# 0beqz/realism-effects

Measured on AMD Instinct MI355X. Metric: Mpixels/s SSGI+denoise @4K steps=20; achieved HBM GB/s vs peak, higher is better.
Workload: dtype f32; 1 GPU; configs[2]: 3840x2160 (8.29 Mpixel) on one GPU, steps=20 refineSteps=5 denoiseIterations=1, K1+K2+2xK3+K4 per step; frame=3840x2160, tile_rows=2160, halo_rows=0, direct_light=True, half_store=rtz, uv_model=reference_gl, parallelism=single GPU

## Files before the change

### realism-effects_amd/csrc/k1_ssgi.hip

```cpp
#include "rfx_brdf.h"
#include "rfx_kernels.h"

namespace {

constexpr int BASE = 16;
constexpr int K1_TH = 1;
typedef uint32_t k1_cell_t;
constexpr int K1_WAVES = 8;
constexpr int K1_COUNTERS = 64;
constexpr int K1_TABLE_CELLS = 9216;
RFX_DEV uint32_t k1_half_toward(float v, bool up) {
    uint32_t h = rfx_f2h_rne(v) & 0xffffu;
    const float f = rfx_h2f((unsigned short)h);
    if (up ? (f < v) : (f > v)) {
        const bool neg = (h & 0x8000u) != 0;
        if (up) h = neg ? (h == 0x8000u ? 0x0001u : h - 1u) : h + 1u;
        else h = neg ? h + 1u : (h == 0x0000u ? 0x8001u : h - 1u);
    }
    return h;
}
RFX_DEV k1_cell_t k1_cell_pack(float mn, float mx) { return k1_half_toward(mn, false) | (k1_half_toward(mx, true) << 16); }
RFX_DEV float2 k1_cell_load(const k1_cell_t *t, unsigned int i) {
    const uint32_t v = *(const k1_cell_t *)((const char *)t + i);
    return make_float2(rfx_h2f((unsigned short)(v & 0xffffu)), rfx_h2f((unsigned short)(v >> 16)));
// ... 599 lines not shown

__global__ __launch_bounds__(256) void k1_hit_mask(FrameDims d, int y0, int y1, TexView depth, TexViewW out, const float4 *hits, int allow_missed, unsigned int *mask) {
    const int x = blockIdx.x * 64 + threadIdx.x, y = y0 + blockIdx.y * 4 + threadIdx.y;
    d.viol = 0;
    if (x >= d.W || y >= y1) return;
    const float dp = ((const float *)depth.ptr)[rfx_xy_index(d, depth.row0, depth.rows, x, y)];
    if (dp == 1.0f) return;
    const size_t i = (size_t)rfx_local_row(d, out.row0, out.rows, y) * d.W + x;
    const float4 h0 = hits[2 * i], h1 = hits[2 * i + 1];
    const float u[2] = {h0.x, h0.z}, v[2] = {h0.y, h0.w}, px[2] = {h1.x, h1.y};
#pragma unroll
    for (int r = 0; r < 2; r++) {
        const bool missed = px[r] == 10.0e9f;
        if ((allow_missed || !missed) && u[r] >= 0.0f && u[r] <= 1.0f && v[r] >= 0.0f && v[r] <= 1.0f) {
            const int row = rfx_nearest_idx(v[r], d.fH, d.H), col = rfx_nearest_idx(u[r], d.fW, d.W);
            const unsigned int bit = 1u << ((unsigned int)(col * 32) / (unsigned int)d.W);
            if (!(mask[row] & bit)) atomicOr(&mask[row], bit);
        }
    }
}

template <int VEC>
__global__ __launch_bounds__(256) void k1_prepare(const float *depth, float *viewz, float2 *base, int W, int H, int base_w, float nearMulFar,
                                                   float farMinusNear, float cameraFar, float nearMinusFar, float cameraNear, int perspective) {
    static_assert(VEC == 1 || VEC == 4, "one texel or one aligned float4 per lane and row");
    const int x0 = (blockIdx.x * 64 + threadIdx.x) * VEC, cy = blockIdx.y * 4 + threadIdx.y, y0 = cy * BASE;
    if (y0 >= H) return;
    float mn = INFINITY, mx = -INFINITY;
    float d[BASE][VEC];
    const bool in_x = x0 < W;
#pragma unroll
    for (int r = 0; r < BASE; r++) {
        const int y = y0 + r;
#pragma unroll
        for (int k = 0; k < VEC; k++) d[r][k] = 1.0f;
        if (in_x && y < H) {
            if (VEC == 4) {
                const float4 t = *(const float4 *)(depth + (size_t)y * W + x0);
                d[r][0] = t.x; d[r][1] = t.y; d[r][2] = t.z; d[r][3] = t.w;
            } else {
                d[r][0] = depth[(size_t)y * W + x0];
            }
        }
    }
#pragma unroll
    for (int r = 0; r < BASE; r++) {
        const int y = y0 + r;
        if (in_x && y < H) {
            float z[VEC];
#pragma unroll
            for (int k = 0; k < VEC; k++) {
                z[k] = perspective ? nearMulFar / (farMinusNear * d[r][k] - cameraFar) : d[r][k] * nearMinusFar - cameraNear;
                mn = fminf(mn, z[k]);
                mx = fmaxf(mx, z[k]);
            }
            if (VEC == 4) *(float4 *)(viewz + (size_t)y * W + x0) = make_float4(z[0], z[1], z[2], z[3]);
            else viewz[(size_t)y * W + x0] = z[0];
        }
    }
#pragma unroll
    for (int o = 1; o < BASE / VEC; o <<= 1) {
        mn = fminf(mn, __shfl_xor(mn, o));
        mx = fmaxf(mx, __shfl_xor(mx, o));
    }
    const int cx = x0 / BASE;
    if ((threadIdx.x & (BASE / VEC - 1)) == 0 && cx < base_w) base[(size_t)cy * base_w + cx] = make_float2(mn, mx);
}

__global__ __launch_bounds__(256) void k1_pack_cells(const float2 *base, int base_w, int base_h, k1_cell_t *cells, int cells_w, int cells_h, int cells_pitch, int up,
                                                     int cells_padded, unsigned int *tile_counter) {
    const int i = blockIdx.x * 256 + threadIdx.x;
    if (i < 64) tile_counter[i * 32] = 0u;
    if (i >= cells_padded) return;
    const int cy = i / cells_pitch, cx = i - cy * cells_pitch;
    if (cy >= cells_h || cx >= cells_w) {
        cells[i] = 0u;
        return;
    }
    float mn = INFINITY, mx = -INFINITY;
    for (int by = cy << up; by < min((cy + 1) << up, base_h); by++)
        for (int bx = cx << up; bx < min((cx + 1) << up, base_w); bx++) {
            const float2 b = base[(size_t)by * base_w + bx];
            mn = fminf(mn, b.x);
            mx = fmaxf(mx, b.y);
        }
    cells[i] = k1_cell_pack(mn, mx);
}

__global__ __launch_bounds__(256) void k1_env_mip(const float4 *src, float4 *dst, int sw, int sh, int dw, int dh, int to_half, int rtz) {
// ... 22 lines not shown
    hipLaunchKernelGGL(k1_env_mip, grid, block, 0, stream, src, dst, sw, sh, dw, dh, to_half ? 1 : 0, rtz ? 1 : 0);
    return hipGetLastError();
}

int rfx_k1_base_cell() { return BASE; }

hipError_t rfx_launch_k1_hit_rows(const FrameDims &d, int y0, int y1, TexView depth, TexViewW out, const float4 *hits, bool allow_missed, int *rows, hipStream_t stream) {
    dim3 block(64, 4), grid((d.W + 63) / 64, (y1 - y0 + 3) / 4);
    hipLaunchKernelGGL(k1_hit_rows, grid, block, 0, stream, d, y0, y1, depth, out, hits, allow_missed ? 1 : 0, rows);
    return hipGetLastError();
}

hipError_t rfx_launch_k1_hit_mask(const FrameDims &d, int y0, int y1, TexView depth, TexViewW out, const float4 *hits, bool allow_missed, unsigned int *mask, hipStream_t stream) {
    dim3 block(64, 4), grid((d.W + 63) / 64, (y1 - y0 + 3) / 4);
    hipLaunchKernelGGL(k1_hit_mask, grid, block, 0, stream, d, y0, y1, depth, out, hits, allow_missed ? 1 : 0, mask);
    return hipGetLastError();
}

hipError_t rfx_launch_k1_prepare(const K1Args &A, hipStream_t stream) {
    const int W = A.dims.W, H = A.dims.H;
    const dim3 block(64, 4);
    if (W % 4 == 0 && ((uintptr_t)A.depth.ptr & 15u) == 0 && ((uintptr_t)A.viewz & 15u) == 0)
        hipLaunchKernelGGL(k1_prepare<4>, dim3((W + 255) / 256, ((H + BASE - 1) / BASE + 3) / 4), block, 0, stream, (const float *)A.depth.ptr, A.viewz, A.coarse, W, H, A.coarse_w,
                           A.nearMulFar, A.farMinusNear, A.p.camera.far_, A.nearMinusFar, A.p.camera.near_, A.p.camera.isPerspective);
    else
        hipLaunchKernelGGL(k1_prepare<1>, dim3((W + 63) / 64, ((H + BASE - 1) / BASE + 3) / 4), block, 0, stream, (const float *)A.depth.ptr, A.viewz, A.coarse, W, H, A.coarse_w,
                           A.nearMulFar, A.farMinusNear, A.p.camera.far_, A.nearMinusFar, A.p.camera.near_, A.p.camera.isPerspective);
    int up = 0;
    while ((BASE << up) < (1 << A.cell_shift)) up++;
    const int padded = A.cells_vec4 * 4;
    hipLaunchKernelGGL(k1_pack_cells, dim3((padded + 255) / 256), dim3(256), 0, stream, (const float2 *)A.coarse, A.coarse_w, A.coarse_h,
                       (k1_cell_t *)A.cells, A.cells_w, A.cells_h, A.cells_pitch, up, padded, A.tile_counter);
    return hipGetLastError();
}

hipError_t rfx_launch_k1(const K1Args &A, int stage, hipStream_t stream) {
    const int nbx = (A.out_w + 63) / 64, nby = (A.y1 - A.y0 + K1_TH - 1) / K1_TH;
    const int want = (nbx * nby + K1_WAVES - 1) / K1_WAVES, n_cu = A.n_cu > 0 ? A.n_cu : 256;
    dim3 block(64 * K1_WAVES), grid(1);
    const float *P = A.p.camera.projectionMatrix;
    const bool persp = P[1] == 0.f && P[2] == 0.f && P[3] == 0.f && P[4] == 0.f && P[6] == 0.f && P[7] == 0.f && P[12] == 0.f && P[13] == 0.f &&
                       P[15] == 0.f && P[11] == -1.f;
    const bool env = A.p.useEnvMap != 0, mis = env && A.p.importanceSampling != 0;
#define K1_GO_S(P, E, M, S)                                                                                                   \
    do {                                                                                                                      \
        static int per_cu[64] = {0};                                                                                          \
        int dev = 0;                                                                                                          \
        hipGetDevice(&dev);                                                                                                   \
        int nb = (dev >= 0 && dev < 64) ? per_cu[dev] : 0;                                                                    \
        if (nb <= 0) {                                                                                                        \
// ... 27 lines not shown
```

### realism-effects_amd/csrc/k3_denoise.hip

```cpp
#include <type_traits>
#include "rfx_device.h"
#include "rfx_kernels.h"
#include "k3_rotation_table.h"

namespace {

constexpr int TW = 64, TH = 8;
constexpr int NT = TW * TH;
static_assert(TW % 64 == 0 && NT <= 1024, "a tile row is whole wavefronts; at most 16 wavefronts per workgroup");
constexpr int K3_XCD_G = 1;
constexpr int K3_LDS_MAX = 80 * 1024;

struct CenterTexel {
    float3 rgb;
    float a;
    float lumaPow;
    float w;
    float total;
};

RFX_DEV float k3_logc(float x) { return rfx_log2(x); }
RFX_DEV float k3_unlog(float o) { return rfx_exp2(o) - 1.0f; }
RFX_DEV float k3_luma(float3 a) {
    return rfx_exp2(__builtin_fmaf(0.125f, rfx_log2(rfx_lum(a)), 0.125f * -0.5287663729448977f));
// ... 22 lines not shown
    const rfx_f2 d = c.lumaPow - tapLuma;
    const rfx_f2 lumaDiff = k3_f2(fminf(fabsf(d.x), 0.5f), fminf(fabsf(d.y), 0.5f));
    const rfx_f2 e = l2w - lumaDiff * lumaPhiL2;
    const rfx_f2 wl = k3_f2(rfx_exp2(e.x), rfx_exp2(e.y));
    rfx_f2 w = (wl * c.omw + disocclW * c.w) * c.w;
    w = k3_f2((w.x < 0.0001f) ? 0.0f : w.x, (w.y < 0.0001f) ? 0.0f : w.y);
    c.r += tr * w;
    c.g += tg * w;
    c.b += tb * w;
    c.total += w;
}
RFX_DEV rfx_f2 k3_logc2(rfx_f2 x) {
    const rfx_f2 x1 = x + 1.0f;
    return k3_f2(rfx_log2(x1.x), rfx_log2(x1.y));
}
RFX_DEV rfx_f2 k3_luma2(rfx_f2 r, rfx_f2 g, rfx_f2 b) {
    const rfx_f2 lum = 0.2125f * r + 0.7154f * g + 0.0721f * b;
    const rfx_f2 l = k3_f2(rfx_log2(lum.x), rfx_log2(lum.y));
    const rfx_f2 e = 0.125f * l + (0.125f * -0.5287663729448977f);
    return k3_f2(rfx_exp2(e.x), rfx_exp2(e.y));
}


template <bool IN_TEMPORAL, int TC, int PITCH, bool WHOLE>
RFX_DEV void k3_tiled_body(const K3Args &A, const FrameDims &d) {
    constexpr bool PAIR = TC == 2;
    extern __shared__ float4 lds[];
    const int Rx = A.tile.Rx, Ry = A.tile.Ry, LW = A.tile.LW, LH = A.tile.LH;
    const int ntex = PITCH * LH;
    float4 *s_geom = lds;
    float4 *s_in0 = lds + ntex;
    uint2 *s_inN = reinterpret_cast<uint2 *>(lds + ntex);
    uint4 *s_in2 = reinterpret_cast<uint4 *>(lds + ntex);
    float *s_depth = reinterpret_cast<float *>(lds + ntex) + (IN_TEMPORAL ? 8 : 4) * (size_t)ntex;
    const int skip = (PAIR && IN_TEMPORAL) ? A.tile.skip : 0;
    if (PAIR && IN_TEMPORAL && skip > 0) {
        const int nal = ntex - 2 * skip;
        s_depth = reinterpret_cast<float *>(lds) + 4 - skip;
        s_geom = lds + 1 + nal / 4 - skip;
        s_in0 = lds + 1 + nal / 4 + nal - 2 * skip;
    }
    const rfx_denoise_params &p = A.p;
    if (PAIR && IN_TEMPORAL && skip > 0) {
        const int t = threadIdx.y * TW + threadIdx.x, nal = ntex - 2 * skip;
        float *f = reinterpret_cast<float *>(lds);
        if (t < 4) f[t] = 0.0f;
        if (t < 8 * skip) f[4 + nal * 13 + t] = 0.0f;
    }
    const TileXY tile = rfx_xcd_tile<K3_XCD_G>((d.W + TW - 1) / TW, (A.y1 - A.y0 + TH - 1) / TH);
    if (!tile.valid) return;
    const int tx0 = tile.bx * TW, ty0 = A.y0 + tile.by * TH;
    const int tid = threadIdx.y * TW + threadIdx.x;
    const float *depthp = (const float *)A.depth.ptr;
    const uint4 *gbp = (const uint4 *)A.gbuffer.ptr;

    const float invLW = 1.0f / (float)LW;
    for (int i = tid; i < LW * LH; i += NT) {
        const int ly = (int)(((float)i + 0.5f) * invLW), lx = i - __mul24(ly, LW);
        const int li = __mul24(ly, PITCH) + lx;
        if (li < skip || li >= ntex - skip) continue;
        const int uy = ty0 - Ry + ly;
        if (uy > A.y1 - 1 + Ry) continue;
        const int gx = min(max(tx0 - Rx + lx, 0), d.W - 1), gy = min(max(uy, 0), d.H - 1);
        const uint4 g = rfx_gather<uint4>(gbp, (unsigned int)(__mul24(rfx_view_row<WHOLE>(d, A.gbuffer, gy), d.W) + gx));
        const float3 n = rfx_unpack_normal(g.y);
        s_geom[li] = make_float4(n.x, n.y, n.z, rfx_decode_roughness(g.z));
        s_depth[li] = rfx_gather<float>(depthp, (unsigned int)(__mul24(rfx_view_row<WHOLE>(d, A.depth, gy), d.W) + gx));
        if constexpr (PAIR && IN_TEMPORAL) {
            float3 l[2];
            float lu[2];
#pragma unroll
            for (int i = 0; i < 2; i++) {
                const TexView &src = p.isTextureSpecular[i] ? A.in1 : A.in0;
                const float4 v = rfx_gather<float4>(src.ptr, (unsigned int)(__mul24(rfx_view_row<WHOLE>(d, src, gy), d.W) + gx));
// ... 194 lines not shown
            c[i].rgb = make_float3(cp2.r[i], cp2.g[i], cp2.b[i]);
            c[i].total = cp2.total[i];
        }
    }

    const size_t oi = (size_t)(unsigned int)(__mul24(WHOLE ? y : rfx_local_row(d, A.out0.row0, A.out0.rows, y), d.W) + x);
#pragma unroll
    for (int i = 0; i < TC; i++) {
        const float inv = rfx_rcp(c[i].total);
        float3 o = make_float3(c[i].rgb.x * inv, c[i].rgb.y * inv, c[i].rgb.z * inv);
        o = make_float3(k3_unlog(o.x), k3_unlog(o.y), k3_unlog(o.z));
        ((uint2 *)(i ? A.out1.ptr : A.out0.ptr))[oi] = rfx_store_half4(o.x, o.y, o.z, c[i].a, p.halfStoreRTZ != 0);
    }
}

template <bool IN_TEMPORAL>
RFX_DEV float4 k3_input(const TexView &t, const FrameDims &d, float u, float v) {
    if (IN_TEMPORAL) return rfx_fetch_f4(t, d, u, v);
    return rfx_fetch_h4_linear(t, d, u, v);
}

template <bool IN_TEMPORAL, int TC>
RFX_DEV void k3_generic_body(const K3Args &A, const FrameDims &d) {
    const int x = blockIdx.x * 64 + threadIdx.x;
    const int y = A.y0 + blockIdx.y * 4 + threadIdx.y;
    if (x >= d.W || y >= A.y1) return;
    const rfx_denoise_params &p = A.p;
    const float u = rfx_frag_u(d.uv, x, y), v = rfx_frag_v(d.uv, y);
    const float *depthp = (const float *)A.depth.ptr;
    const uint4 *gbp = (const uint4 *)A.gbuffer.ptr;
    const float depth = depthp[rfx_xy_index(d, A.depth.row0, A.depth.rows, x, y)];
    const int qx0 = x & ~1, qx1 = x | 1, qy0 = y & ~1, qy1 = y | 1;
    {
        float dxa = depthp[rfx_xy_index(d, A.depth.row0, A.depth.rows, qx0, y)], dxb = depthp[rfx_xy_index(d, A.depth.row0, A.depth.rows, qx1, y)];
        float dya = depthp[rfx_xy_index(d, A.depth.row0, A.depth.rows, x, qy0)], dyb = depthp[rfx_xy_index(d, A.depth.row0, A.depth.rows, x, qy1)];
        if (depth == 1.0f && (fabsf(dxb - dxa) + fabsf(dyb - dya)) == 0.0f) return;
    }
    CenterTexel c[TC];
    bool isSpec[TC];
#pragma unroll
    for (int i = 0; i < TC; i++) {
        isSpec[i] = p.isTextureSpecular[i] != 0;
        float4 t = k3_input<IN_TEMPORAL>(isSpec[i] ? A.in1 : A.in0, d, u, v);
        c[i].w = 1.0f / rfx_pow(t.w + 1.0f, 1.2f * p.phi);
        const float3 col = k3_log3(t.x * 1.0003f, t.y * 1.0003f, t.z * 1.0003f);
        c[i].rgb = col;
// ... 95 lines not shown
    A.tile.Ry = k3_apron(ry);
    A.tile.LW = TW + 2 * A.tile.Rx;
    A.tile.LH = TH + 2 * A.tile.Ry;
    A.tile.skip = 0;
    const int pitch = A.tile.LW <= TW + 8 ? TW + 8 : A.tile.LW <= TW + 10 ? TW + 10 : A.tile.LW <= TW + 12 ? TW + 12 : A.tile.LW <= TW + 16 ? TW + 16 : A.tile.LW <= TW + 32 ? TW + 32 : 0;
    size_t lds = (size_t)pitch * A.tile.LH * (16 + 4 + 2 * (temporal ? 16 : 8));
    if (temporal && A.p.textureCount == 2 && pitch == A.tile.LW && pitch != 0) {
        const float t = ((float)A.tile.Ry - 0.5f - SLACK) / ry;
        const int X = (int)floorf(0.5f + rx * sqrtf(fmaxf(0.0f, 1.0f - t * t)) + SLACK);
        int skip = A.tile.Rx - X;
        if (skip > 4) skip = 4;
        const int ntex = pitch * A.tile.LH;
        while (skip > 0 && ((ntex - 2 * skip) & 3) != 0) skip--;
        if (skip > 0) {
            A.tile.skip = skip;
            lds = 16 + (size_t)(ntex - 2 * skip) * (4 + 16 + 32) + (size_t)skip * 32;
        }
    }
    const bool tiled = A.p.radius >= 0.0f && pitch != 0 && lds <= (size_t)K3_LDS_MAX;
    const auto whole_view = [&](const void *ptr, int row0, int rows) { return ptr == nullptr || (row0 == 0 && rows == A.dims.H); };
    const bool whole = whole_view(A.depth.ptr, A.depth.row0, A.depth.rows) && whole_view(A.gbuffer.ptr, A.gbuffer.row0, A.gbuffer.rows) &&
                       whole_view(A.in0.ptr, A.in0.row0, A.in0.rows) && whole_view(A.in1.ptr, A.in1.row0, A.in1.rows) &&
                       whole_view(A.out0.ptr, A.out0.row0, A.out0.rows) && whole_view(A.out1.ptr, A.out1.row0, A.out1.rows);
    if (tiled) {
        dim3 block(TW, TH), grid(rfx_xcd_grid(K3_XCD_G, (A.dims.W + TW - 1) / TW, (A.y1 - A.y0 + TH - 1) / TH));
#define K3_TILED(T, C, P, WH)                                                                                                \
    do {                                                                                                                     \
        static bool attr_set[64] = {false};                                                                                  \
        int dev = 0;                                                                                                         \
        hipGetDevice(&dev);                                                                                                  \
        if (dev < 0 || dev >= 64 || !attr_set[dev]) {                                                                        \
            hipFuncSetAttribute((const void *)k3_tiled<T, C, P, WH>, hipFuncAttributeMaxDynamicSharedMemorySize, K3_LDS_MAX); \
            if (dev >= 0 && dev < 64) attr_set[dev] = true;                                                                  \
        }                                                                                                                    \
        hipLaunchKernelGGL((k3_tiled<T, C, P, WH>), grid, block, lds, stream, A);                                            \
    } while (0)
#define K3_TILED_W(T, C, P) do { if (whole) K3_TILED(T, C, P, true); else K3_TILED(T, C, P, false); } while (0)
#define K3_TILED_P(T, C)                    \
    do {                                    \
        if (pitch == TW + 8) K3_TILED_W(T, C, TW + 8); \
        else if (pitch == TW + 10) K3_TILED_W(T, C, TW + 10); \
        else if (pitch == TW + 12) K3_TILED_W(T, C, TW + 12); \
        else if (pitch == TW + 16) K3_TILED_W(T, C, TW + 16); \
        else K3_TILED_W(T, C, TW + 32);          \
    } while (0)
        if (A.p.textureCount == 2) {
// ... 22 lines not shown
```

### realism-effects_amd/csrc/rfx_api.hip

```cpp
#include <hip/hip_runtime.h>
#include <stdio.h>
#include <stdlib.h>
#include <string.h>
#include <string>
#include "../../include/rfx.h"
#include "rfx_kernels.h"

#include "rfx_ctx.h"

thread_local std::string g_create_err;

#define RFX_ENTER(c) hipSetDevice((c)->device)
static hipEvent_t prof_event(rfx_ctx *c) {
    hipEvent_t e = nullptr;
    if (!c->prof_free.empty()) { e = c->prof_free.back(); c->prof_free.pop_back(); return e; }
    return hipEventCreate(&e) == hipSuccess ? e : nullptr;
}
static void prof_recycle(rfx_ctx *c) {
    for (const rfx_ctx::ProfRec &r : c->prof_recs) { c->prof_free.push_back(r.a); c->prof_free.push_back(r.b); }
    c->prof_recs.clear();
}
struct ProfScope {
    rfx_ctx *c;
    hipStream_t stream;
// ... 78 lines not shown
    if (c->upload_stream) { hipStreamSynchronize(c->upload_stream); hipStreamDestroy(c->upload_stream); }
    for (int i = 0; i < RFX_TEX_COUNT; i++) {
        if (c->slots[i].owned && c->slots[i].ptr) hipFree(c->slots[i].ptr);
        if (c->slots[i].back) hipFree(c->slots[i].back);
    }
    for (hipEvent_t e : c->ev_batch)
        if (e) hipEventDestroy(e);
    if (c->ev_staged) hipEventDestroy(c->ev_staged);
    if (c->ev_frame_done) hipEventDestroy(c->ev_frame_done);
    if (c->halo_violations) hipFree(c->halo_violations);
    if (c->viewz) hipFree(c->viewz);
    if (c->prep_stream) { hipStreamSynchronize(c->prep_stream); hipStreamDestroy(c->prep_stream); }
    for (hipEvent_t e : {c->ev_depth, c->ev_k1_done, c->ev_prep_done})
        if (e) hipEventDestroy(e);
    if (c->hits) hipFree(c->hits);
    if (c->hit_rows_dev) hipFree(c->hit_rows_dev);
    if (c->hit_rows_host) hipHostFree(c->hit_rows_host);
    if (c->hit_mask_dev) hipFree(c->hit_mask_dev);
    if (c->hit_mask_host) hipHostFree(c->hit_mask_host);
    if (c->hist_staging) hipFree(c->hist_staging);
    if (c->coarse) hipFree(c->coarse);
    if (c->cells) hipFree(c->cells);
    if (c->k1_tiles) hipFree(c->k1_tiles);
    if (c->env) hipFree(c->env);
    if (c->env_marginal) hipFree(c->env_marginal);
    if (c->env_conditional) hipFree(c->env_conditional);
    prof_recycle(c);
    for (hipEvent_t e : c->prof_free) hipEventDestroy(e);
    if (c->ev0) hipEventDestroy(c->ev0);
    if (c->ev1) hipEventDestroy(c->ev1);
    if (c->own_stream) hipStreamDestroy(c->own_stream);
    delete c;
}

const char *rfx_last_error(const rfx_ctx *c) { return c ? c->err.c_str() : g_create_err.c_str(); }

int rfx_get_geometry(const rfx_ctx *c, int *width, int *height, int *tile_y0, int *tile_rows, int *halo_rows) {
    if (!c) return RFX_EINVAL;
    if (width) *width = c->W;
    if (height) *height = c->H;
    if (tile_y0) *tile_y0 = c->tile_y0;
    if (tile_rows) *tile_rows = c->tile_rows;
    if (halo_rows) *halo_rows = c->halo;
    return RFX_OK;
}

// ... 38 lines not shown
    e = hipMemsetAsync(s.ptr, 0, bytes, c->stream);
    if (e != hipSuccess) return fail(c, RFX_EDEVICE, "hipMemsetAsync", e);
    return RFX_OK;
}

static int band_check(rfx_ctx *c, int id, int row0, int rows) {
    if (id < 0 || id >= RFX_TEX_COUNT) return fail(c, RFX_EINVAL, "bad texture id");
    const Slot &s = c->slots[id];
    if (rows <= 0 || row0 < s.row0 || row0 + rows > s.row0 + s.rows) return fail(c, RFX_EINVAL, "row band outside the rows this context holds");
    return RFX_OK;
}

int rfx_upload(rfx_ctx *c, rfx_tex id, const void *host, int row0, int rows) {
    if (!c || !host) return RFX_EINVAL;
    int rc = band_check(c, id, row0, rows);
    if (rc) return rc;
    if ((rc = ensure(c, id))) return rc;
    RFX_ENTER(c);
    Slot &s = c->slots[id];
    const size_t pitch = (size_t)s.width * s.texel;
    HIPCHK(c, hipMemcpyAsync((char *)s.ptr + (size_t)(row0 - s.row0) * pitch, host, (size_t)rows * pitch, hipMemcpyHostToDevice, c->stream));
    HIPCHK(c, hipStreamSynchronize(c->stream));
    s.uploaded = true;
    if (id == RFX_TEX_DEPTH) c->depth_event_set = false;
    return RFX_OK;
}

int rfx_download(rfx_ctx *c, rfx_tex id, void *host, int row0, int rows) {
    if (!c || !host) return RFX_EINVAL;
    int rc = band_check(c, id, row0, rows);
    if (rc) return rc;
    if ((rc = ensure(c, id))) return rc;
    RFX_ENTER(c);
    Slot &s = c->slots[id];
    const size_t pitch = (size_t)s.width * s.texel;
    HIPCHK(c, hipMemcpyAsync(host, (char *)s.ptr + (size_t)(row0 - s.row0) * pitch, (size_t)rows * pitch, hipMemcpyDeviceToHost, c->stream));
    HIPCHK(c, hipStreamSynchronize(c->stream));
    return RFX_OK;
}

void *rfx_host_alloc(size_t bytes) {
    void *p = nullptr;
    return hipHostMalloc(&p, bytes, hipHostMallocDefault) == hipSuccess ? p : nullptr;
}
void rfx_host_free(void *p) {
    if (p) hipHostFree(p);
}
// ... 25 lines not shown
    }
    HIPCHK(c, hipStreamWaitEvent(c->upload_stream, c->ev_frame_done, 0));
    HIPCHK(c, hipMemcpyAsync((char *)s.back + (size_t)(row0 - s.row0) * pitch, host, (size_t)rows * pitch, hipMemcpyHostToDevice, c->upload_stream));
    s.back_filled = true;
    return RFX_OK;
}

int rfx_stage_flip(rfx_ctx *c) {
    if (!c) return RFX_EINVAL;
    if (!c->upload_stream) return fail(c, RFX_ESTATE, "rfx_stage_flip: nothing staged");
    RFX_ENTER(c);
    HIPCHK(c, hipEventRecord(c->ev_staged, c->upload_stream));
    HIPCHK(c, hipStreamWaitEvent(c->stream, c->ev_staged, 0));
    HIPCHK(c, hipEventRecord(c->ev_frame_done, c->stream));
    const unsigned int k = c->flips++;
    HIPCHK(c, hipEventRecord(c->ev_batch[k & 1], c->upload_stream));
    if (k >= 1) HIPCHK(c, hipEventSynchronize(c->ev_batch[(k - 1) & 1]));
    for (int id = 0; id < RFX_TEX_COUNT; id++) {
        Slot &s = c->slots[id];
        if (!s.back_filled) continue;
        if (id == RFX_TEX_DEPTH) {
            HIPCHK(c, hipEventRecord(c->ev_depth, c->upload_stream));
            c->depth_event_set = true;
        }
        void *t = s.ptr; s.ptr = s.back; s.back = t;
        s.back_filled = false;
        s.uploaded = true;
    }
    return RFX_OK;
}

int rfx_clear(rfx_ctx *c, rfx_tex id) {
    if (!c || id < 0 || id >= RFX_TEX_COUNT) return RFX_EINVAL;
    int rc = ensure(c, id);
    if (rc) return rc;
    RFX_ENTER(c);
    Slot &s = c->slots[id];
    HIPCHK(c, hipMemsetAsync(s.ptr, 0, (size_t)s.rows * s.width * s.texel, c->stream));
    if (id == RFX_TEX_DEPTH) {
        HIPCHK(c, hipEventRecord(c->ev_depth, c->stream));
        c->depth_event_set = true;
    }
    return RFX_OK;
}

void *rfx_tex_device_ptr(rfx_ctx *c, rfx_tex id) {
    if (!c || id < 0 || id >= RFX_TEX_COUNT) return nullptr;
    hipSetDevice(c->device);
    if (ensure(c, id)) return nullptr;
    if (id == RFX_TEX_DEPTH) c->depth_external = true;
    return c->slots[id].ptr;
}

int rfx_bind_external(rfx_ctx *c, rfx_tex id, void *device_ptr) {
    if (!c || id < 0 || id >= RFX_TEX_COUNT || !device_ptr) return RFX_EINVAL;
    RFX_ENTER(c);
    Slot &s = c->slots[id];
    if (s.owned && s.ptr) {
        HIPCHK(c, hipStreamSynchronize(c->stream));
        hipFree(s.ptr);
    }
    s.ptr = device_ptr;
    s.owned = false;
    s.uploaded = true;
    if (id == RFX_TEX_DEPTH) c->depth_external = true;
    return RFX_OK;
}

static TexView view(rfx_ctx *c, int id) {
    TexView v;
    v.ptr = c->slots[id].ptr; v.row0 = c->slots[id].row0; v.rows = c->slots[id].rows;
    return v;
}
static TexViewW wview(rfx_ctx *c, int id) {
    TexViewW v;
    v.ptr = c->slots[id].ptr; v.row0 = c->slots[id].row0; v.rows = c->slots[id].rows;
    return v;
}
static UvPlanes rfx_uv_planes(int model, int w, int h) {
    UvPlanes q;
    q.model = model; q.W = w; q.H = h; q.fW = (float)w; q.fH = (float)h;
    const float ooa = 1.0f / ((float)w * (float)h);
    q.du = (float)h * ooa;
    q.dv = (float)w * ooa;
    const float far_u = q.du * ((float)w - 0.5f), far_v = q.dv * ((float)h - 0.5f);
    q.u0_upper = 0.5f * q.du;
    q.u0_lower = 1.0f - far_u;
    q.v0 = 1.0f - far_v;
// ... 273 lines not shown
            while ((1 << pitch_log2) < cw) pitch_log2++;
            pitch = 1 << pitch_log2;
        }
        return (size_t)((pitch * ch + 3) / 4) * 16;
    };
    A.cells_pow2 = 0;
    for (A.cell_shift = 4;; A.cell_shift++) {
        if (k1_table(A.cell_shift, false, A.cells_w, A.cells_h, A.cells_pitch, A.cells_pitch_log2) <= (size_t)table_budget || A.cell_shift >= 12) break;
    }
    if (RFX_K1_POW2) {
        int cw, ch, pitch, pl2;
        if (k1_table(A.cell_shift, true, cw, ch, pitch, pl2) <= (size_t)table_budget) {
            A.cells_pow2 = 1;
            A.cells_pitch = pitch;
            A.cells_pitch_log2 = pl2;
        }
    }
    A.cells_vec4 = (A.cells_pitch * A.cells_h + 3) / 4;
    if (!c->viewz) {
        hipError_t e = hipMalloc((void **)&c->viewz, (size_t)c->W * c->H * sizeof(float));
        if (e == hipSuccess) e = hipMalloc((void **)&c->coarse, (size_t)A.coarse_w * A.coarse_h * sizeof(float2));
        if (e == hipSuccess) e = hipMalloc((void **)&c->cells, (size_t)A.cells_vec4 * 16);
        if (e == hipSuccess) e = hipMalloc((void **)&c->k1_tiles, 64 * 128);
        if (e != hipSuccess) {
            if (c->viewz) hipFree(c->viewz);
            if (c->coarse) hipFree(c->coarse);
            if (c->cells) hipFree(c->cells);
            if (c->k1_tiles) hipFree(c->k1_tiles);
            c->viewz = nullptr; c->coarse = nullptr; c->cells = nullptr; c->k1_tiles = nullptr;
            return fail(c, RFX_ENOMEM, "hipMalloc(K1 scratch)", e);
        }
    }
    A.viewz = c->viewz;
    A.coarse = c->coarse;
    A.cells = c->cells;
    A.tile_counter = c->k1_tiles;
    A.n_cu = c->n_cu;
    A.env = c->env;
    A.env_w = c->env_w; A.env_h = c->env_h; A.env_levels = c->env_levels;
    A.env_marginal = c->env_marginal; A.env_conditional = c->env_conditional;
    A.totalSumWhole = c->env_sum_whole; A.totalSumDecimal = c->env_sum_decimal;
    memcpy(A.env_off, c->env_off, sizeof A.env_off);
    {
        int m = c->env_w > c->env_h ? c->env_w : c->env_h, lg = 0;
        while ((m >> (lg + 1)) > 0) lg++;
        A.maxEnvMapMipLevel = c->env ? (float)(lg + 1) : 0.0f;
    }
    A.hits = nullptr;
    if (stage != 0) {
        const size_t n = (size_t)c->W * c->slots[RFX_TEX_SSGI].rows * 2;
        if (stage == 2 && (!c->hits || !c->hits_traced))
            return fail(c, RFX_ESTATE, "rfx_ssgi_shade: no rfx_ssgi_trace of this frame to finish");
        if (!c->hits) {
            hipError_t e = hipMalloc((void **)&c->hits, n * sizeof(float4));
            if (e != hipSuccess) return fail(c, RFX_ENOMEM, "hipMalloc(K1 trace hand-over)", e);
        }
        A.hits = c->hits;
    }
    if (stage != 2) {
#ifndef RFX_K1_PREP_STREAM
#define RFX_K1_PREP_STREAM 1
#endif
        if (c->depth_external || !RFX_K1_PREP_STREAM) {
            ProfScope prof(c, RFX_PROF_K1_PREPASS, c->stream);
            HIPCHK(c, rfx_launch_k1_prepare(A, c->stream));
        } else {
            if (c->depth_event_set) HIPCHK(c, hipStreamWaitEvent(c->prep_stream, c->ev_depth, 0));
            if (c->k1_event_set) HIPCHK(c, hipStreamWaitEvent(c->prep_stream, c->ev_k1_done, 0));
            {
                ProfScope prof(c, RFX_PROF_K1_PREPASS, c->prep_stream);
                HIPCHK(c, rfx_launch_k1_prepare(A, c->prep_stream));
            }
            HIPCHK(c, hipEventRecord(c->ev_prep_done, c->prep_stream));
            HIPCHK(c, hipStreamWaitEvent(c->stream, c->ev_prep_done, 0));
        }
    }
    if (any && stage == 2) HIPCHK(c, hipMemsetAsync(c->k1_tiles, 0, 64 * 128, c->stream));
    if (any) {
        ProfScope prof(c, RFX_PROF_K1_MARCH, c->stream);
        HIPCHK(c, rfx_launch_k1(A, stage, c->stream));
    }
    HIPCHK(c, hipEventRecord(c->ev_k1_done, c->stream));
    c->k1_event_set = true;
    c->hits_traced = stage == 1;
    if (stage == 1) { c->trace_y0 = A.y0; c->trace_y1 = any ? A.y1 : A.y0; c->trace_missed = p->missedRays; c->trace_scaled = rs != 1.0f; }
    return RFX_OK;
}

int rfx_internal_hit_rows_enqueue(rfx_ctx *c, int *rows_dev) {
    if (!c->hits || !c->hits_traced) return fail(c, RFX_ESTATE, "rfx_gather_history_rows: no rfx_ssgi_trace of this frame is waiting for its shade");
    if (c->trace_scaled) return fail(c, RFX_EUNSUPPORTED, "rfx_ssgi_hit_rows / rfx_gather_history_rows: the last rfx_ssgi_trace ran with resolutionScale != 1");
    RFX_ENTER(c);
    static const int preset[2] = {0x7fffffff, -1};
    HIPCHK(c, hipMemcpyAsync(rows_dev, preset, sizeof preset, hipMemcpyHostToDevice, c->stream));
    if (c->trace_y1 > c->trace_y0)
        HIPCHK(c, rfx_launch_k1_hit_rows(dims(c), c->trace_y0, c->trace_y1, view(c, RFX_TEX_DEPTH), wview(c, RFX_TEX_SSGI), c->hits, c->trace_missed != 0, rows_dev, c->stream));
    return RFX_OK;
}
// ... 116 lines not shown
int rfx_poisson_denoise(rfx_ctx *c, const rfx_denoise_params *p) {
    if (!c || !p) return RFX_EINVAL;
    if (p->textureCount != 1 && p->textureCount != 2) return fail(c, RFX_EINVAL, "rfx_poisson_denoise: textureCount");
    RFX_ENTER(c);
    const int in0 = p->inputIsTemporal ? RFX_TEX_TEMPORAL0 : (p->writeToB ? RFX_TEX_DENOISE_A0 : RFX_TEX_DENOISE_B0);
    const int in1 = p->inputIsTemporal ? RFX_TEX_TEMPORAL1 : (p->writeToB ? RFX_TEX_DENOISE_A1 : RFX_TEX_DENOISE_B1);
    const int out0 = p->writeToB ? RFX_TEX_DENOISE_B0 : RFX_TEX_DENOISE_A0;
    const int out1 = p->writeToB ? RFX_TEX_DENOISE_B1 : RFX_TEX_DENOISE_A1;
    const int ids[] = {RFX_TEX_DEPTH, RFX_TEX_GBUFFER, RFX_TEX_BLUE_NOISE, in0, in1, out0, out1};
    int rc = need(c, ids, 7);
    if (rc) return rc;
    if (!c->slots[RFX_TEX_DEPTH].uploaded || !c->slots[RFX_TEX_GBUFFER].uploaded || !c->slots[RFX_TEX_BLUE_NOISE].uploaded)
        return fail(c, RFX_ESTATE, "rfx_poisson_denoise: depth / gbuffer / blue-noise not uploaded");
    K3Args A;
    A.dims = dims(c);
    if (!launch_rows(c, out0, 0, &A.y0, &A.y1)) return RFX_OK;
    A.depth = view(c, RFX_TEX_DEPTH); A.gbuffer = view(c, RFX_TEX_GBUFFER);
    A.in0 = view(c, in0);
    A.in1 = view(c, p->textureCount == 2 ? in1 : in0);
    A.blue = c->slots[RFX_TEX_BLUE_NOISE].ptr;
    blue_noise_shift(p->blueNoiseIndex, &A.shift_x, &A.shift_y);
    A.out0 = wview(c, out0); A.out1 = wview(c, out1);
    A.p = *p;
    ProfScope prof(c, p->inputIsTemporal ? RFX_PROF_K3_PASS0 : RFX_PROF_K3_PASSN, c->stream);
    HIPCHK(c, rfx_launch_k3(A, c->stream));
    return RFX_OK;
}

int rfx_compose(rfx_ctx *c, const rfx_compose_params *p) {
    if (!c || !p) return RFX_EINVAL;
    if (p->inputType != 0 && p->inputType != 2)
        return fail(c, RFX_EUNSUPPORTED, "rfx_compose: inputType diffuseSpecular (0) and specular (2) are built");
    RFX_ENTER(c);
    if (p->giSource != 0 && p->giSource != 1) return fail(c, RFX_EINVAL, "rfx_compose: giSource");
    const int g0 = p->giSource ? RFX_TEX_TEMPORAL0 : RFX_TEX_DENOISE_B0, g1 = p->giSource ? RFX_TEX_TEMPORAL1 : RFX_TEX_DENOISE_B1;
    const int ids[] = {RFX_TEX_DEPTH, RFX_TEX_GBUFFER, g0, g1, RFX_TEX_COMPOSE, RFX_TEX_DIRECT_LIGHT};
    int rc = need(c, ids, 6);
    if (rc) return rc;
    K4Args A;
    A.dims = dims(c);
    launch_rows(c, RFX_TEX_COMPOSE, 0, &A.y0, &A.y1);
    if (A.y0 < c->tile_y0) A.y0 = c->tile_y0;
    if (A.y1 > c->tile_y0 + c->tile_rows) A.y1 = c->tile_y0 + c->tile_rows;
    const bool any = A.y1 > A.y0;
    A.depth = view(c, RFX_TEX_DEPTH); A.gbuffer = view(c, RFX_TEX_GBUFFER);
    A.gi0 = view(c, g0); A.gi1 = view(c, g1);
// ... 156 lines not shown
```

### realism-effects_amd/csrc/rfx_ctx.h

```cpp
#pragma once
#include <hip/hip_runtime.h>
#include <stdio.h>
#include <string>
#include <vector>
#include "../../include/rfx.h"

struct Slot {
    void *ptr = nullptr;
    bool owned = false;
    int row0 = 0, rows = 0;
    size_t texel = 0;
    int width = 0;
    bool uploaded = false;
    void *back = nullptr;
    bool back_filled = false;
};

struct rfx_ctx {
    int device = 0;
    int W = 0, H = 0, tile_y0 = 0, tile_rows = 0, halo = 0;
    hipStream_t own_stream = nullptr, stream = nullptr;
    hipEvent_t ev0 = nullptr, ev1 = nullptr;
    unsigned int *halo_violations = nullptr;
    float *viewz = nullptr;
    float4 *hits = nullptr;
    bool hits_traced = false;
    int trace_y0 = 0, trace_y1 = 0, trace_missed = 0;
    bool trace_scaled = false;
    int *hit_rows_dev = nullptr;
    int *hit_rows_host = nullptr;
    unsigned int *hit_mask_dev = nullptr, *hit_mask_host = nullptr;
    int hit_mask_ranks = 0;
    void *hist_staging = nullptr;
    size_t hist_staging_bytes = 0;
    hipStream_t prep_stream = nullptr;
    hipEvent_t ev_depth = nullptr, ev_k1_done = nullptr, ev_prep_done = nullptr;
    bool depth_event_set = false, k1_event_set = false, depth_external = false;
    int win_y0 = 0, win_y1 = 0x7fffffff;
    int uv_model = RFX_UV_REFERENCE_GL;
    float2 *coarse = nullptr;
    unsigned int *cells = nullptr;
    unsigned int *k1_tiles = nullptr;
    int n_cu = 0;
    float4 *env = nullptr;
    float *env_marginal = nullptr, *env_conditional = nullptr;
    float env_sum_whole = 1.0f, env_sum_decimal = 0.0f;
    int env_w = 0, env_h = 0, env_levels = 0;
    unsigned int env_off[16] = {0};
    Slot slots[RFX_TEX_COUNT];
    void *comm = nullptr;
    bool comm_owned = false;
    int comm_rank = 0, comm_nranks = 1;
    hipStream_t comm_stream = nullptr;
    hipEvent_t ev_draws = nullptr, ev_comm = nullptr;
    bool comm_pending = false;
    hipStream_t upload_stream = nullptr;
    hipEvent_t ev_staged = nullptr, ev_frame_done = nullptr;
    hipEvent_t ev_batch[2] = {nullptr, nullptr};
    unsigned int flips = 0;
    unsigned long long *peer_flags = nullptr;
    void **peer_table_dev = nullptr;
    unsigned long long *peer_status_dev = nullptr, *peer_status_host = nullptr;
    std::vector<void *> peer_mapped;
    hipEvent_t ev_peer_release = nullptr;
    bool peer_release_pending = false;
    int peer_n = 0, peer_rank = 0, peer_tex = -1;
// ... 41 lines not shown
```

### realism-effects_amd/csrc/rfx_kernels.h

```cpp
#pragma once
#include <hip/hip_runtime.h>
#include "rfx_device.h"


#ifndef RFX_K1_POW2
#define RFX_K1_POW2 1
#endif
struct K1Args {
    FrameDims dims;
    int y0, y1;
    TexView depth, gbuffer, direct, history;
    const void *blue;
    int shift_x, shift_y;
    TexViewW out;
    rfx_ssgi_params p;
    float nearMulFar, farMinusNear, nearMinusFar;
    float *viewz;
    float2 *coarse;
    int coarse_w, coarse_h;
    unsigned int *cells;
    int cells_w, cells_h, cell_shift, cells_vec4;
    int cells_pitch, cells_pitch_log2;
    int cells_pow2;
    const float4 *env;
    int env_w, env_h, env_levels;
    unsigned int env_off[16];
    float maxEnvMapMipLevel;
    const float *env_marginal, *env_conditional;
    float totalSumWhole, totalSumDecimal;
    int out_w, out_h;
    UvPlanes out_uv;
    float4 *hits;
    unsigned int *tile_counter;
    int n_cu;
};

hipError_t rfx_launch_env_mip(const float4 *src, float4 *dst, int sw, int sh, int dw, int dh, bool to_half, bool rtz, hipStream_t);

struct K2Args {
    FrameDims dims;
    int y0, y1;
    TexView ssgi, velocity, hist0, hist1;
    int hist_f32;
    int in_w, in_h;
    TexViewW out0, out1;
    rfx_temporal_params p;
    float invW, invH;
    float rcpInvW, rcpInvH;
    float prevPV[16];
};

struct K3Args {
    FrameDims dims;
    int y0, y1;
    TexView depth, gbuffer, in0, in1;
    const void *blue;
    int shift_x, shift_y;
    TexViewW out0, out1;
    rfx_denoise_params p;
    struct { int Rx, Ry, LW, LH, skip; } tile;
    float tap_ox[8], tap_oy[8];
};

struct K4Args {
    FrameDims dims;
    int y0, y1;
    TexView depth, gbuffer, gi0, gi1;
    TexView scene;
    TexViewW out;
    float *rgb_out;
    rfx_compose_params p;
};

hipError_t rfx_launch_pack_gbuffer(int W, int rows, const float *diffuse, const float *normal, const float *roughness, const float *metalness,
                                   const float *emissive, const float *depth, void *out, hipStream_t);
hipError_t rfx_launch_pack_velocity(int W, int rows, const float *velocity, const float *normal, const float *depth, void *out, hipStream_t);
hipError_t rfx_launch_cube_to_equirect(float4 *chain, int size, int levels, float4 *out, int W, int H, const UvPlanes &uv, hipStream_t);

struct K5Args {
    FrameDims dims;
    int y0, y1;
    TexView depth, gi, scene;
    TexViewW out;
    rfx_final_params p;
// ... 31 lines not shown
```

Baseline: 6579 Mpixels/s.

## Skip background tiles in denoise using a foreground map built in K1 prepare

k1_prepare now also writes a per-64x8-tile byte map marking tiles that contain any pixel whose depth is not 1.0. The map is double-buffered and tagged with a depth generation counter. K3 denoise blocks (tiled and generic) read this map and return early for tiles with no foreground pixels, saving the depth, gbuffer and history loads and the filtering work there. In exchange, k1_prepare does a little extra shuffle and store work, and the skip is only correct if denoise writes nothing needed for sky pixels and the tile geometry matches the map granularity.

```diff
diff --git a/realism-effects_amd/csrc/k1_ssgi.hip b/realism-effects_amd/csrc/k1_ssgi.hip
--- a/realism-effects_amd/csrc/k1_ssgi.hip
+++ b/realism-effects_amd/csrc/k1_ssgi.hip
@@ -645,7 +645,8 @@
 
 template <int VEC>
 __global__ __launch_bounds__(256) void k1_prepare(const float *depth, float *viewz, float2 *base, int W, int H, int base_w, float nearMulFar,
-                                                   float farMinusNear, float cameraFar, float nearMinusFar, float cameraNear, int perspective) {
+                                                   float farMinusNear, float cameraFar, float nearMinusFar, float cameraNear, int perspective,
+                                                   unsigned char *fg, int fg_w) {
     static_assert(VEC == 1 || VEC == 4, "one texel or one aligned float4 per lane and row");
     const int x0 = (blockIdx.x * 64 + threadIdx.x) * VEC, cy = blockIdx.y * 4 + threadIdx.y, y0 = cy * BASE;
     if (y0 >= H) return;
@@ -688,6 +689,16 @@
     }
     const int cx = x0 / BASE;
     if ((threadIdx.x & (BASE / VEC - 1)) == 0 && cx < base_w) base[(size_t)cy * base_w + cx] = make_float2(mn, mx);
+    static_assert(BASE == 16, "a strip is two 8-row map tiles high");
+    int any = 0;
+#pragma unroll
+    for (int r = 0; r < BASE; r++)
+#pragma unroll
+        for (int k = 0; k < VEC; k++) any |= (d[r][k] != 1.0f ? 1 : 0) << (r >> 3);
+#pragma unroll
+    for (int o = 1; o < 64 / VEC; o <<= 1) any |= __shfl_xor(any, o);
+    const int h = threadIdx.x & (64 / VEC - 1), tx = x0 >> 6, ty = 2 * cy + h;
+    if (h < 2 && tx < fg_w && ty * 8 < H) fg[(size_t)ty * fg_w + tx] = (unsigned char)((any >> h) & 1);
 }
 
 __global__ __launch_bounds__(256) void k1_pack_cells(const float2 *base, int base_w, int base_h, k1_cell_t *cells, int cells_w, int cells_h, int cells_pitch, int up,
@@ -756,10 +767,10 @@
     const dim3 block(64, 4);
     if (W % 4 == 0 && ((uintptr_t)A.depth.ptr & 15u) == 0 && ((uintptr_t)A.viewz & 15u) == 0)
         hipLaunchKernelGGL(k1_prepare<4>, dim3((W + 255) / 256, ((H + BASE - 1) / BASE + 3) / 4), block, 0, stream, (const float *)A.depth.ptr, A.viewz, A.coarse, W, H, A.coarse_w,
-                           A.nearMulFar, A.farMinusNear, A.p.camera.far_, A.nearMinusFar, A.p.camera.near_, A.p.camera.isPerspective);
+                           A.nearMulFar, A.farMinusNear, A.p.camera.far_, A.nearMinusFar, A.p.camera.near_, A.p.camera.isPerspective, A.fg_tiles, A.fg_w);
     else
         hipLaunchKernelGGL(k1_prepare<1>, dim3((W + 63) / 64, ((H + BASE - 1) / BASE + 3) / 4), block, 0, stream, (const float *)A.depth.ptr, A.viewz, A.coarse, W, H, A.coarse_w,
-                           A.nearMulFar, A.farMinusNear, A.p.camera.far_, A.nearMinusFar, A.p.camera.near_, A.p.camera.isPerspective);
+                           A.nearMulFar, A.farMinusNear, A.p.camera.far_, A.nearMinusFar, A.p.camera.near_, A.p.camera.isPerspective, A.fg_tiles, A.fg_w);
     int up = 0;
     while ((BASE << up) < (1 << A.cell_shift)) up++;
     const int padded = A.cells_vec4 * 4;
diff --git a/realism-effects_amd/csrc/k3_denoise.hip b/realism-effects_amd/csrc/k3_denoise.hip
--- a/realism-effects_amd/csrc/k3_denoise.hip
+++ b/realism-effects_amd/csrc/k3_denoise.hip
@@ -68,6 +68,13 @@
 }
 
 
+RFX_DEV bool k3_tile_is_background(const K3Args &A, const FrameDims &d, int bx, int y0) {
+    if (!A.fg_tiles) return false;
+    const unsigned int i = (unsigned int)((y0 >> 3) * ((d.W + 63) >> 6) + bx);
+    const unsigned int w = reinterpret_cast<const unsigned int *>(A.fg_tiles)[i >> 2];
+    return ((w >> ((i & 3u) * 8u)) & 0xffu) == 0u;
+}
+
 template <bool IN_TEMPORAL, int TC, int PITCH, bool WHOLE>
 RFX_DEV void k3_tiled_body(const K3Args &A, const FrameDims &d) {
     constexpr bool PAIR = TC == 2;
@@ -87,15 +94,16 @@
         s_in0 = lds + 1 + nal / 4 + nal - 2 * skip;
     }
     const rfx_denoise_params &p = A.p;
+    const TileXY tile = rfx_xcd_tile<K3_XCD_G>((d.W + TW - 1) / TW, (A.y1 - A.y0 + TH - 1) / TH);
+    if (!tile.valid) return;
+    const int tx0 = tile.bx * TW, ty0 = A.y0 + tile.by * TH;
+    if (k3_tile_is_background(A, d, tile.bx, ty0)) return;
     if (PAIR && IN_TEMPORAL && skip > 0) {
         const int t = threadIdx.y * TW + threadIdx.x, nal = ntex - 2 * skip;
         float *f = reinterpret_cast<float *>(lds);
         if (t < 4) f[t] = 0.0f;
         if (t < 8 * skip) f[4 + nal * 13 + t] = 0.0f;
     }
-    const TileXY tile = rfx_xcd_tile<K3_XCD_G>((d.W + TW - 1) / TW, (A.y1 - A.y0 + TH - 1) / TH);
-    if (!tile.valid) return;
-    const int tx0 = tile.bx * TW, ty0 = A.y0 + tile.by * TH;
     const int tid = threadIdx.y * TW + threadIdx.x;
     const float *depthp = (const float *)A.depth.ptr;
     const uint4 *gbp = (const uint4 *)A.gbuffer.ptr;
@@ -336,6 +344,7 @@
 
 template <bool IN_TEMPORAL, int TC>
 RFX_DEV void k3_generic_body(const K3Args &A, const FrameDims &d) {
+    if (k3_tile_is_background(A, d, blockIdx.x, A.y0 + blockIdx.y * 4)) return;
     const int x = blockIdx.x * 64 + threadIdx.x;
     const int y = A.y0 + blockIdx.y * 4 + threadIdx.y;
     if (x >= d.W || y >= A.y1) return;
@@ -477,6 +486,7 @@
     const bool whole = whole_view(A.depth.ptr, A.depth.row0, A.depth.rows) && whole_view(A.gbuffer.ptr, A.gbuffer.row0, A.gbuffer.rows) &&
                        whole_view(A.in0.ptr, A.in0.row0, A.in0.rows) && whole_view(A.in1.ptr, A.in1.row0, A.in1.rows) &&
                        whole_view(A.out0.ptr, A.out0.row0, A.out0.rows) && whole_view(A.out1.ptr, A.out1.row0, A.out1.rows);
+    if (!whole) A.fg_tiles = nullptr;
     if (tiled) {
         dim3 block(TW, TH), grid(rfx_xcd_grid(K3_XCD_G, (A.dims.W + TW - 1) / TW, (A.y1 - A.y0 + TH - 1) / TH));
 #define K3_TILED(T, C, P, WH)                                                                                                \
diff --git a/realism-effects_amd/csrc/rfx_api.hip b/realism-effects_amd/csrc/rfx_api.hip
--- a/realism-effects_amd/csrc/rfx_api.hip
+++ b/realism-effects_amd/csrc/rfx_api.hip
@@ -124,6 +124,7 @@
     if (c->coarse) hipFree(c->coarse);
     if (c->cells) hipFree(c->cells);
     if (c->k1_tiles) hipFree(c->k1_tiles);
+    if (c->fg_tiles) hipFree(c->fg_tiles);
     if (c->env) hipFree(c->env);
     if (c->env_marginal) hipFree(c->env_marginal);
     if (c->env_conditional) hipFree(c->env_conditional);
@@ -208,7 +209,10 @@
     HIPCHK(c, hipMemcpyAsync((char *)s.ptr + (size_t)(row0 - s.row0) * pitch, host, (size_t)rows * pitch, hipMemcpyHostToDevice, c->stream));
     HIPCHK(c, hipStreamSynchronize(c->stream));
     s.uploaded = true;
-    if (id == RFX_TEX_DEPTH) c->depth_event_set = false;
+    if (id == RFX_TEX_DEPTH) {
+        c->depth_event_set = false;
+        c->depth_gen++;
+    }
     return RFX_OK;
 }
 
@@ -280,6 +284,7 @@
         if (id == RFX_TEX_DEPTH) {
             HIPCHK(c, hipEventRecord(c->ev_depth, c->upload_stream));
             c->depth_event_set = true;
+            c->depth_gen++;
         }
         void *t = s.ptr; s.ptr = s.back; s.back = t;
         s.back_filled = false;
@@ -298,6 +303,7 @@
     if (id == RFX_TEX_DEPTH) {
         HIPCHK(c, hipEventRecord(c->ev_depth, c->stream));
         c->depth_event_set = true;
+        c->depth_gen++;
     }
     return RFX_OK;
 }
@@ -306,7 +312,7 @@
     if (!c || id < 0 || id >= RFX_TEX_COUNT) return nullptr;
     hipSetDevice(c->device);
     if (ensure(c, id)) return nullptr;
-    if (id == RFX_TEX_DEPTH) c->depth_external = true;
+    if (id == RFX_TEX_DEPTH) { c->depth_external = true; c->depth_gen++; }
     return c->slots[id].ptr;
 }
 
@@ -321,7 +327,7 @@
     s.ptr = device_ptr;
     s.owned = false;
     s.uploaded = true;
-    if (id == RFX_TEX_DEPTH) c->depth_external = true;
+    if (id == RFX_TEX_DEPTH) { c->depth_external = true; c->depth_gen++; }
     return RFX_OK;
 }
 
@@ -641,12 +647,16 @@
         if (e == hipSuccess) e = hipMalloc((void **)&c->coarse, (size_t)A.coarse_w * A.coarse_h * sizeof(float2));
         if (e == hipSuccess) e = hipMalloc((void **)&c->cells, (size_t)A.cells_vec4 * 16);
         if (e == hipSuccess) e = hipMalloc((void **)&c->k1_tiles, 64 * 128);
+        c->fg_w = (c->W + 63) / 64;
+        c->fg_stride = (((size_t)c->fg_w * ((c->H + 7) / 8)) + 255) & ~(size_t)255;
+        if (e == hipSuccess) e = hipMalloc((void **)&c->fg_tiles, 2 * c->fg_stride);
         if (e != hipSuccess) {
             if (c->viewz) hipFree(c->viewz);
             if (c->coarse) hipFree(c->coarse);
             if (c->cells) hipFree(c->cells);
             if (c->k1_tiles) hipFree(c->k1_tiles);
-            c->viewz = nullptr; c->coarse = nullptr; c->cells = nullptr; c->k1_tiles = nullptr;
+            if (c->fg_tiles) hipFree(c->fg_tiles);
+            c->viewz = nullptr; c->coarse = nullptr; c->cells = nullptr; c->k1_tiles = nullptr; c->fg_tiles = nullptr;
             return fail(c, RFX_ENOMEM, "hipMalloc(K1 scratch)", e);
         }
     }
@@ -655,6 +665,9 @@
     A.cells = c->cells;
     A.tile_counter = c->k1_tiles;
     A.n_cu = c->n_cu;
+    const int fg_next = c->fg_cur ^ 1;
+    A.fg_tiles = c->fg_tiles + (size_t)fg_next * c->fg_stride;
+    A.fg_w = c->fg_w;
     A.env = c->env;
     A.env_w = c->env_w; A.env_h = c->env_h; A.env_levels = c->env_levels;
     A.env_marginal = c->env_marginal; A.env_conditional = c->env_conditional;
@@ -693,6 +706,8 @@
             HIPCHK(c, hipEventRecord(c->ev_prep_done, c->prep_stream));
             HIPCHK(c, hipStreamWaitEvent(c->stream, c->ev_prep_done, 0));
         }
+        c->fg_cur = fg_next;
+        c->fg_gen = c->depth_gen;
     }
     if (any && stage == 2) HIPCHK(c, hipMemsetAsync(c->k1_tiles, 0, 64 * 128, c->stream));
     if (any) {
@@ -855,6 +870,7 @@
     blue_noise_shift(p->blueNoiseIndex, &A.shift_x, &A.shift_y);
     A.out0 = wview(c, out0); A.out1 = wview(c, out1);
     A.p = *p;
+    A.fg_tiles = (c->fg_tiles && c->fg_gen == c->depth_gen && !c->depth_external && (A.y0 & 7) == 0) ? c->fg_tiles + (size_t)c->fg_cur * c->fg_stride : nullptr;
     ProfScope prof(c, p->inputIsTemporal ? RFX_PROF_K3_PASS0 : RFX_PROF_K3_PASSN, c->stream);
     HIPCHK(c, rfx_launch_k3(A, c->stream));
     return RFX_OK;
diff --git a/realism-effects_amd/csrc/rfx_ctx.h b/realism-effects_amd/csrc/rfx_ctx.h
--- a/realism-effects_amd/csrc/rfx_ctx.h
+++ b/realism-effects_amd/csrc/rfx_ctx.h
@@ -42,6 +42,10 @@
     unsigned int *cells = nullptr;
     unsigned int *k1_tiles = nullptr;
     int n_cu = 0;
+    unsigned char *fg_tiles = nullptr;
+    size_t fg_stride = 0;
+    int fg_w = 0, fg_cur = 0;
+    unsigned long long depth_gen = 1, fg_gen = 0;
     float4 *env = nullptr;
     float *env_marginal = nullptr, *env_conditional = nullptr;
     float env_sum_whole = 1.0f, env_sum_decimal = 0.0f;
diff --git a/realism-effects_amd/csrc/rfx_kernels.h b/realism-effects_amd/csrc/rfx_kernels.h
--- a/realism-effects_amd/csrc/rfx_kernels.h
+++ b/realism-effects_amd/csrc/rfx_kernels.h
@@ -33,6 +33,8 @@
     float4 *hits;
     unsigned int *tile_counter;
     int n_cu;
+    unsigned char *fg_tiles;
+    int fg_w;
 };
 
 hipError_t rfx_launch_env_mip(const float4 *src, float4 *dst, int sw, int sh, int dw, int dh, bool to_half, bool rtz, hipStream_t);
@@ -60,6 +62,7 @@
     rfx_denoise_params p;
     struct { int Rx, Ry, LW, LH, skip; } tile;
     float tap_ox[8], tap_oy[8];
+    const unsigned char *fg_tiles;
 };
 
 struct K4Args {
```

Result: faster. 6672 Mpixels/s (median of 6 runs) (+1.4%).
